# nintendops/DynamicFusion_Body

Measured on AMD Instinct MI355X. Metric: Mvoxels/s TSDF fusion + GN-iters/s warp solve, 256³ grid, 1/2/4/8 GPU, higher is better.
Workload: dtype f64 geometry / f32 volume

## Files before the change

### dynamicfusion_body_amd/csrc/dfh_integrate.hip

```cpp
#include "dfh_common.h"

#include <cstdlib>

namespace dfh {

template <typename T, int N>
struct alignas(sizeof(T) * N) Pack {
    T v[N];
};

struct IntegrateParams {
    Mat3 K, Kinv;
    Mat34 lw;
    double scale, cx, cy, cz, half, tdist, wmax;
    double Ax[4], Ay[4], Az[4], Ac[4];
    double inv_scale;
    float tdist_f, ts_f, wmax_f;
    int zp_shift;
    int planes_per_block;
    int X, Y, Z;
    int x0, nx;
    int H, W;
    int zpacks;
    const float *pyr;
    int pyr_off[6], pyr_w[6], pyr_h[6];
    int cull;
};

constexpr int kFixShift = 20;
constexpr int kFixOne = 1 << kFixShift;
constexpr int kFixHalf = 1 << (kFixShift - 1);
constexpr int kFixBand = 8;
constexpr int kFastMaxDim = 2048;
constexpr int kBrX = 4, kBrY = 2, kBrZ = 256 / (kBrX * kBrY);
constexpr int kMaxColumnBricks = 16;
constexpr int kPyrLevels = 5;
constexpr int kCullMargin = 1 << 10;
constexpr long kEarlyRowsMaxVoxels = 1L << 23;
constexpr long kTargetBlocks = 1L << 40;

template <typename DepthT, bool PINHOLE>
__device__ __forceinline__ bool exact_voxel(const IntegrateParams &p, const DepthT *__restrict__ depth,
                                            int x, int y, int z, double &sd_out) {
    const double *lw = p.lw.m;
    const double px = p.scale * ((double)x - p.half) + p.cx;
    const double py = p.scale * ((double)y - p.half) + p.cy;
    const double pz = p.scale * ((double)z - p.half) + p.cz;
    const double l0 = ((lw[0] * px + lw[1] * py) + lw[2] * pz) + lw[3];
    const double l1 = ((lw[4] * px + lw[5] * py) + lw[6] * pz) + lw[7];
    const double l2 = ((lw[8] * px + lw[9] * py) + lw[10] * pz) + lw[11];
    double p0, p1, p2;
    if (PINHOLE) {
        p0 = p.K.m[0] * l0 + p.K.m[2] * l2;
        p1 = p.K.m[4] * l1 + p.K.m[5] * l2;
        p2 = l2;
    } else {
        p0 = (p.K.m[0] * l0 + p.K.m[1] * l1) + p.K.m[2] * l2;
        p1 = (p.K.m[3] * l0 + p.K.m[4] * l1) + p.K.m[5] * l2;
        p2 = (p.K.m[6] * l0 + p.K.m[7] * l1) + p.K.m[8] * l2;
    }
    sd_out = 0.0;
    if (!(p2 != 0.0)) return false;
    const double u = p0 / p2;
    const double v = p1 / p2;
    if (!((u >= 0.0) && (u < (double)(p.W - 1)) && (v >= 0.0) && (v < (double)(p.H - 1)))) return false;
    const int ui = (int)rint(u);
    const int vi = (int)rint(v);
    const double zd = -1.0 * (double)depth[(size_t)vi * p.W + ui];
    if (!(zd > 0.0)) return false;
    double cz;
    if (PINHOLE) {
        cz = zd;
    } else {
        cz = (p.Kinv.m[6] * (zd * u) + p.Kinv.m[7] * (zd * v)) + p.Kinv.m[8] * (zd * 1.0);
    }
    const double sd = cz - l2;
    sd_out = sd;
    return sd > -1.0 * p.tdist;
}

template <typename DepthT, bool PINHOLE, bool LAZY>
__device__ __forceinline__ bool exact_voxel_rare(const IntegrateParams *pp, const DepthT *__restrict__ depth,
                                                 int x, int y, int z, double &sd_out) {
    asm volatile("" : "+v"(x), "+v"(y), "+v"(z));
    if (LAZY) asm volatile("" : "+s"(pp));
    return exact_voxel<DepthT, PINHOLE>(*pp, depth, x, y, z, sd_out);
}

__device__ __forceinline__ const IntegrateParams *kernarg_params(int byte_offset) {
    typedef const char __attribute__((address_space(4))) *KernArgBytes;
    KernArgBytes ka = (KernArgBytes)__builtin_amdgcn_kernarg_segment_ptr();
    return (const IntegrateParams *)(ka + byte_offset);
}
constexpr int kParamsAfterThreePointers = 24;

__device__ __forceinline__ double rcp_nr1(double d) {
    const double r = __builtin_amdgcn_rcp(d);
    return __builtin_fma(r, __builtin_fma(-d, r, 1.0), r);
}

__device__ __forceinline__ int cvt_i32_sat(double x) {
    int r;
    asm("v_cvt_i32_f64 %0, %1" : "=v"(r) : "v"(x));
    return r;
}

__device__ __forceinline__ void pack_coords(const IntegrateParams &p, int &y, int &zp) {
    const int lin = blockIdx.x * 256 + threadIdx.x;
    if (p.zp_shift >= 0) {
        y = lin >> p.zp_shift;
        zp = lin & ((1 << p.zp_shift) - 1);
    } else {
        y = lin / p.zpacks;
        zp = lin - y * p.zpacks;
    }
}

struct NoHook {
    __device__ __forceinline__ void operator()(bool) const {}
};

template <typename DepthT, int VEC, bool PINHOLE, bool STRIDED, bool LAZY = true, typename Hook = NoHook>
__device__ __forceinline__ bool view_pack(const IntegrateParams &p, const IntegrateParams *p_rare, const DepthT *__restrict__ depth, int x,
                                          int y, int z0, float (&ms)[VEC], bool (&upd)[VEC], Hook &&after_gathers = NoHook()) {
    constexpr int ZS = STRIDED ? 64 : 1;
    constexpr int NC = PINHOLE ? 3 : 4;
    const unsigned ulim = (unsigned)(p.W - 1) << kFixShift;
    const unsigned vlim = (unsigned)(p.H - 1) << kFixShift;
    double base[NC];
    {
        const double xf = (double)x, yf = (double)y, zf = (double)z0;
#pragma unroll
        for (int r = 0; r < NC; ++r)
            base[r] = __builtin_fma(p.Az[r], zf, __builtin_fma(p.Ax[r], xf, __builtin_fma(p.Ay[r], yf, p.Ac[r])));
    }
    const double p2_last = __builtin_fma(p.Az[2], (double)((VEC - 1) * ZS), base[2]);
    const bool pack_singular = !((fabs(base[2]) > 1e-6) & (fabs(p2_last) > 1e-6) & ((base[2] > 0.0) == (p2_last > 0.0)));

    double l2v[VEC];
    float l2f[VEC];
    unsigned pix[VEC];
    bool inside[VEC], amb[VEC];
    double rinv[VEC];
    if (VEC == 4) {
        double d[4];
#pragma unroll
        for (int j = 0; j < 4; ++j) d[j] = __builtin_fma(p.Az[2], (double)(j * ZS), base[2]);
        const double d01 = d[0] * d[1], d23 = d[2] * d[3];
        const double rall = rcp_nr1(d01 * d23);
        const double r01 = rall * d23, r23 = rall * d01;
        rinv[0] = r01 * d[1]; rinv[1] = r01 * d[0]; rinv[2 % VEC] = r23 * d[3 % VEC]; rinv[3 % VEC] = r23 * d[2 % VEC];
    } else {
#pragma unroll
        for (int j = 0; j < VEC; ++j) rinv[j] = rcp_nr1(__builtin_fma(p.Az[2], (double)(j * ZS), base[2]));
    }
#pragma unroll
    for (int j = 0; j < VEC; ++j) {
        const double jf = (double)(j * ZS);
        const double p0 = __builtin_fma(p.Az[0], jf, base[0]);
        const double p1 = __builtin_fma(p.Az[1], jf, base[1]);
        const double p2 = __builtin_fma(p.Az[2], jf, base[2]);
        l2v[j] = PINHOLE ? p2 : __builtin_fma(p.Az[NC - 1], jf, base[NC - 1]);
        l2f[j] = (float)l2v[j];
        const double r = rinv[j];
        const int qu = cvt_i32_sat(p0 * r);
        const int qv = cvt_i32_sat(p1 * r);
        const unsigned du = (unsigned)((qu + kFixBand) & (kFixHalf - 1));
        const unsigned dv = (unsigned)((qv + kFixBand) & (kFixHalf - 1));
        amb[j] = pack_singular | ((du < dv ? du : dv) <= 2u * kFixBand);
        inside[j] = ((unsigned)qu < ulim) & ((unsigned)qv < vlim);
        const int ui = (qu + kFixHalf) >> kFixShift;
        const int vi = (qv + kFixHalf) >> kFixShift;
        pix[j] = inside[j] ? (unsigned)(__mul24(vi, p.W) + ui) : 0u;
    }
    DepthT dval[VEC];
#pragma unroll
    for (int j = 0; j < VEC; ++j) dval[j] = depth[pix[j]];
    {
        bool any_inside = false;
#pragma unroll
        for (int j = 0; j < VEC; ++j) any_inside = any_inside | inside[j] | amb[j];
        after_gathers(any_inside);
    }
    bool any = false;
#pragma unroll
    for (int j = 0; j < VEC; ++j) {
        const float zdf = -(float)dval[j];
        const bool hit = inside[j] & (zdf > 0.0f);
        bool ok, redo, freespace;
        if (PINHOLE) {
            const float d32 = zdf - (l2f[j] - p.tdist_f);
            const float band = fmaf(fabsf(l2f[j]), 2e-6f, 1e-5f);
            ok = hit & (d32 > 0.0f);
            redo = amb[j] | (hit & (fabsf(d32) <= band));
            freespace = d32 > 2.0f * p.tdist_f + band;
        } else {
            ok = hit;
            redo = amb[j];
            freespace = false;
        }
        float m = p.ts_f;
        if (__builtin_expect(redo, 0)) {
            double sd;
            ok = exact_voxel_rare<DepthT, PINHOLE, LAZY>(p_rare, depth, x, y, z0 + j * ZS, sd);
            m = (float)((sd < p.tdist ? sd : p.tdist) * p.inv_scale);
        } else if (ok & !freespace) {
            double cz = -(double)dval[j];
            if (!PINHOLE) {
                const double jf = (double)(j * ZS);
                const double r = rcp_nr1(__builtin_fma(p.Az[2], jf, base[2])) * (1.0 / (double)kFixOne);
                const double u = __builtin_fma(p.Az[0], jf, base[0]) * r;
                const double v = __builtin_fma(p.Az[1], jf, base[1]) * r;
                cz = __builtin_fma(p.Kinv.m[6] * cz, u, __builtin_fma(p.Kinv.m[7] * cz, v, p.Kinv.m[8] * cz));
            }
            const double sd = cz - l2v[j];
            if (!PINHOLE) {
                const double margin = sd + p.tdist;
                ok = margin > 0.0;
                if (fabs(margin) < 1e-7) ok = exact_voxel_rare<DepthT, PINHOLE, LAZY>(p_rare, depth, x, y, z0 + j * ZS, cz);
            }
            m = (float)((sd < p.tdist ? sd : p.tdist) * p.inv_scale);
        }
        ok = ok & (z0 + j * ZS < p.Z);
        ms[j] = m;
        upd[j] = ok;
        any = any | ok;
    }
    return any;
}

template <int VEC>
__device__ __forceinline__ void apply_pack(Pack<float, VEC> &t, Pack<float, VEC> &w, const float (&ms)[VEC], const bool (&upd)[VEC],
                                           float wmax_f) {
#pragma unroll
    for (int j = 0; j < VEC; ++j) {
        const float wt = w.v[j];
        const float d = wt + 1.0f;
        const float n = fmaf(t.v[j], wt, ms[j]);
        const float r = __builtin_amdgcn_rcpf(d);
        float q = n * r;
        q = fmaf(fmaf(-d, q, n), r, q);
        t.v[j] = upd[j] ? q : t.v[j];
        w.v[j] = upd[j] ? fminf(d, wmax_f) : wt;
    }
}

template <typename DepthT, int VEC, bool PINHOLE, bool STRIDED>
__global__ __launch_bounds__(256) void integrate_depth_kernel(float *__restrict__ tsdf,
                                                               float *__restrict__ tsdf_w,
                                                               const DepthT *__restrict__ depth,
                                                               const IntegrateParams p) {
    int y, zp;
    pack_coords(p, y, zp);
    if (y >= p.Y) return;
    const int lane = threadIdx.x & 63;
    const int z0 = STRIDED ? (zp - lane) * VEC + lane : zp * VEC;
    constexpr int ZS = STRIDED ? 64 : 1;
    const int xl_end = min(p.nx, (int)(blockIdx.y + 1) * p.planes_per_block);
    for (int xl = blockIdx.y * p.planes_per_block; xl < xl_end; ++xl) {
        float ms[VEC];
        bool upd[VEC];
        if (!view_pack<DepthT, VEC, PINHOLE, STRIDED>(p, kernarg_params(kParamsAfterThreePointers), depth, p.x0 + xl, y, z0, ms, upd)) continue;
        const size_t off = ((size_t)xl * p.Y + y) * p.Z + z0;
        using P = Pack<float, VEC>;
        P t, w;
        if (STRIDED) {
#pragma unroll
            for (int j = 0; j < VEC; ++j) { t.v[j] = tsdf[off + j * ZS]; w.v[j] = tsdf_w[off + j * ZS]; }
        } else {
            t = *reinterpret_cast<const P *>(tsdf + off);
            w = *reinterpret_cast<const P *>(tsdf_w + off);
        }
        apply_pack<VEC>(t, w, ms, upd, p.wmax_f);
        if (STRIDED) {
#pragma unroll
            for (int j = 0; j < VEC; ++j) {
                if (upd[j]) { tsdf[off + j * ZS] = t.v[j]; tsdf_w[off + j * ZS] = w.v[j]; }
            }
        } else {
            *reinterpret_cast<P *>(tsdf + off) = t;
            *reinterpret_cast<P *>(tsdf_w + off) = w;
        }
    }
}

template <typename DepthT, bool PINHOLE>
__global__ __launch_bounds__(256) void integrate_depth_rows_early_kernel(float *__restrict__ tsdf, float *__restrict__ tsdf_w,
                                                                          const DepthT *__restrict__ depth, const IntegrateParams p) {
    int y, zp;
    pack_coords(p, y, zp);
    if (y >= p.Y) return;
    const int z0 = zp * 4;
    const int xl = blockIdx.y;
    float ms[4];
    bool upd[4];
    const size_t off = ((size_t)xl * p.Y + y) * p.Z + z0;
    using P = Pack<float, 4>;
    P t, w;
    bool loaded = false;
    const bool any = view_pack<DepthT, 4, PINHOLE, false>(p, kernarg_params(kParamsAfterThreePointers), depth, p.x0 + xl, y, z0, ms, upd, [&](bool any_inside) {
        if (any_inside) {
            t = *reinterpret_cast<const P *>(tsdf + off);
            w = *reinterpret_cast<const P *>(tsdf_w + off);
            loaded = true;
        }
    });
    if (!any) return;
    if (!loaded) {
        t = *reinterpret_cast<const P *>(tsdf + off);
        w = *reinterpret_cast<const P *>(tsdf_w + off);
    }
    apply_pack<4>(t, w, ms, upd, p.wmax_f);
    *reinterpret_cast<P *>(tsdf + off) = t;
    *reinterpret_cast<P *>(tsdf_w + off) = w;
}

constexpr int kMaxViews = 16;
struct ViewPtrs {
    const void *depth[kMaxViews];
    int n;
};

template <typename DepthT, int VEC, bool PINHOLE>
__global__ __launch_bounds__(256) void integrate_depth_multi_kernel(float *__restrict__ tsdf, float *__restrict__ tsdf_w,
                                                                     const IntegrateParams *__restrict__ views, const ViewPtrs vp) {
    int y, zp;
    pack_coords(views[0], y, zp);
    if (y >= views[0].Y) return;
    const int z0 = zp * VEC;
    const int nx = views[0].nx, ppb = views[0].planes_per_block;
    const int xl_end = min(nx, (int)(blockIdx.y + 1) * ppb);
    for (int xl = blockIdx.y * ppb; xl < xl_end; ++xl) {
        using P = Pack<float, VEC>;
        P t, w;
        bool loaded = false;
        const size_t off = ((size_t)xl * views[0].Y + y) * views[0].Z + z0;
        for (int v = 0; v < vp.n; ++v) {
            const IntegrateParams &p = views[v];
            float ms[VEC];
            bool upd[VEC];
            if (!view_pack<DepthT, VEC, PINHOLE, false, false>(p, &p, static_cast<const DepthT *>(vp.depth[v]), p.x0 + xl, y, z0, ms, upd)) continue;
            if (!loaded) {
                t = *reinterpret_cast<const P *>(tsdf + off);
                w = *reinterpret_cast<const P *>(tsdf_w + off);
                loaded = true;
            }
            apply_pack<VEC>(t, w, ms, upd, p.wmax_f);
        }
        if (loaded) {
            *reinterpret_cast<P *>(tsdf + off) = t;
            *reinterpret_cast<P *>(tsdf_w + off) = w;
        }
    }
}


struct BrickGeom {
    int nbz;
    int nyb;
    int nxb;
    int nzi;
    int nzc;
};

struct BrickBounds {
    int umin, umax, vmin, vmax;
    double l2min;
    bool front;
};

template <bool PINHOLE, int BY>
__device__ __forceinline__ void brick_corner(const IntegrateParams &p, int x0, int y0, int z0, int c, int &qu, int &qv, double &l2, bool &front) {
    constexpr int NC = PINHOLE ? 3 : 4;
    constexpr int BZ = 256 / (kBrX * BY);
    const double xf = (double)(x0 + ((c & 1) ? kBrX - 1 : 0)), yf = (double)(y0 + ((c & 2) ? BY - 1 : 0)), zf = (double)(z0 + ((c & 4) ? BZ - 1 : 0));
    double q[NC];
#pragma unroll
    for (int r = 0; r < NC; ++r) q[r] = __builtin_fma(p.Az[r], zf, __builtin_fma(p.Ax[r], xf, __builtin_fma(p.Ay[r], yf, p.Ac[r])));
    front = q[2] > 1e-6;
    const double rr = rcp_nr1(q[2]);
    qu = cvt_i32_sat(q[0] * rr);
    qv = cvt_i32_sat(q[1] * rr);
    l2 = q[NC - 1];
}

template <bool PINHOLE>
__device__ __forceinline__ bool bounds_culled(const IntegrateParams &p, BrickBounds b) {
    if (!b.front) return false;
    int umin = b.umin, umax = b.umax, vmin = b.vmin, vmax = b.vmax;
    const int ulim = (p.W - 1) << kFixShift, vlim = (p.H - 1) << kFixShift;
    if (umax < -kCullMargin || umin > ulim + kCullMargin || vmax < -kCullMargin || vmin > vlim + kCullMargin) return true;
    if (!PINHOLE || p.pyr == nullptr) return false;
    umin = max(umin, -2 * kFixOne); vmin = max(vmin, -2 * kFixOne);
    umax = min(umax, ulim + 2 * kFixOne); vmax = min(vmax, vlim + 2 * kFixOne);
    int px0 = (umin - kCullMargin) >> kFixShift, px1 = (umax + kCullMargin + kFixOne - 1) >> kFixShift;
    int py0 = (vmin - kCullMargin) >> kFixShift, py1 = (vmax + kCullMargin + kFixOne - 1) >> kFixShift;
    px0 = max(px0, 0); py0 = max(py0, 0); px1 = min(px1, p.W - 1); py1 = min(py1, p.H - 1);
    if (px1 < px0 || py1 < py0) return false;
    int L = 1;
    while (L <= kPyrLevels && (((px1 >> L) - (px0 >> L)) > 1 || ((py1 >> L) - (py0 >> L)) > 1)) ++L;
    if (L > kPyrLevels) {
        L = kPyrLevels;
        if (((px1 >> L) - (px0 >> L)) > 3 || ((py1 >> L) - (py0 >> L)) > 3) return false;
    }
    const float *lv = p.pyr + p.pyr_off[L];
    const int wl = p.pyr_w[L];
    const int cx0 = px0 >> L, cx1 = px1 >> L, cy0 = py0 >> L, cy1 = py1 >> L;
    float zmax = 0.0f;
    for (int cy = cy0; cy <= cy1; ++cy)
        for (int cx = cx0; cx <= cx1; ++cx) zmax = fmaxf(zmax, lv[cy * wl + cx]);
    const float l2f = (float)b.l2min;
    return zmax + p.tdist_f + fmaf(fabsf(l2f), 4e-7f, 1e-5f) <= l2f;
}

template <bool PINHOLE, int BY>
__device__ __forceinline__ bool brick_culled(const IntegrateParams &p, int x0, int y0, int z0) {
    BrickBounds b{0x7fffffff, (int)0x80000000, 0x7fffffff, (int)0x80000000, __builtin_huge_val(), true};
#pragma unroll
    for (int c = 0; c < 8; ++c) {
        int qu, qv;
        double l2;
        bool fr;
        brick_corner<PINHOLE, BY>(p, x0, y0, z0, c, qu, qv, l2, fr);
        b.front = b.front && fr;
        b.umin = min(b.umin, qu); b.umax = max(b.umax, qu); b.vmin = min(b.vmin, qv); b.vmax = max(b.vmax, qv);
        b.l2min = fmin(b.l2min, l2);
    }
    return bounds_culled<PINHOLE>(p, b);
}

template <bool PINHOLE, bool BYVAL, int BY>
__global__ __launch_bounds__(256) void brick_classify_kernel(const IntegrateParams *__restrict__ views, const IntegrateParams p1,
                                                              int n_views, const BrickGeom g, int n_bricks,
                                                              unsigned short *__restrict__ mask) {
    constexpr int BZ = 256 / (kBrX * BY);
    const int b = blockIdx.x * 256 + threadIdx.x;
    if (b >= n_bricks) return;
    const int bz = b % g.nbz;
    const int t = b / g.nbz;
    const int by = t % g.nyb;
    const int bx = t / g.nyb;
    unsigned m = 0;
    for (int v = 0; v < n_views; ++v) {
        const IntegrateParams &p = BYVAL ? p1 : views[v];
        if (!(p.cull && brick_culled<PINHOLE, BY>(p, p.x0 + kBrX * bx, BY * by, BZ * bz))) m |= 1u << v;
    }
    mask[b] = (unsigned short)m;
}

typedef float f32x4 __attribute__((ext_vector_type(4)));
static_assert(sizeof(f32x4) == sizeof(Pack<float, 4>), "a pack is one 16-byte access");

template <bool NT>
__device__ __forceinline__ Pack<float, 4> ld_pack(const float *a) {
    const f32x4 v = NT ? __builtin_nontemporal_load(reinterpret_cast<const f32x4 *>(a)) : *reinterpret_cast<const f32x4 *>(a);
    Pack<float, 4> r;
    r.v[0] = v.x; r.v[1] = v.y; r.v[2] = v.z; r.v[3] = v.w;
    return r;
}
template <bool NT>
__device__ __forceinline__ void st_pack(float *a, const Pack<float, 4> &r) {
    f32x4 v;
    v.x = r.v[0]; v.y = r.v[1]; v.z = r.v[2]; v.w = r.v[3];
    if (NT) __builtin_nontemporal_store(v, reinterpret_cast<f32x4 *>(a));
    else *reinterpret_cast<f32x4 *>(a) = v;
}

template <int BY>
struct ColumnLane {
    static constexpr int BZ = 256 / (kBrX * BY), BZP = BZ / 4;
    int xl, y, zl, bz0;
    bool in_xy;
    size_t row;
    unsigned mv;

    __device__ __forceinline__ unsigned long long init(const BrickGeom &g, int nx, int Y, int Z, const unsigned short *__restrict__ mask,
                                                       unsigned full_mask, bool all) {
        const int lane = threadIdx.x & 63;
        const int wv = __builtin_amdgcn_readfirstlane((int)(threadIdx.x >> 6));
        const int by = blockIdx.x, c = blockIdx.y, bx = blockIdx.z;
        xl = kBrX * bx + lane / (BY * BZP);
        y = BY * by + (lane / BZP) % BY;
        zl = 4 * (lane % BZP);
        bz0 = 4 * c * g.nzi + wv;
        in_xy = xl < nx && y < Y;
        row = ((size_t)xl * Y + y) * Z;
        const int bz = bz0 + 4 * lane;
        const bool mine = lane < g.nzi && bz < g.nbz;
        mv = 0;
        if (mine) mv = mask ? (unsigned)mask[(size_t)(bx * g.nyb + by) * g.nbz + bz] : full_mask;
        return __ballot(all ? mine : mv != 0);
    }

    __device__ __forceinline__ int z_of(int i) const { return BZ * (bz0 + 4 * i) + zl; }
};

#ifndef DFH_K1_GF_WAVES
#define DFH_K1_GF_WAVES 7
#endif
#ifdef DFH_K1_WAVES
#define DFH_K1_OCC __attribute__((amdgpu_waves_per_eu(DFH_K1_WAVES, DFH_K1_WAVES)))
#else
#define DFH_K1_OCC __attribute__((amdgpu_waves_per_eu(GATHER_FIRST && PINHOLE ? DFH_K1_GF_WAVES : 1)))
#endif
template <typename DepthT, bool PINHOLE, int BY, bool PREFETCH, bool NT, bool GATHER_FIRST>
__global__ __launch_bounds__(256) DFH_K1_OCC void integrate_depth_column_kernel(float *__restrict__ tsdf, float *__restrict__ tsdf_w,
                                                                      const DepthT *__restrict__ depth, const IntegrateParams p,
                                                                      const BrickGeom g, const unsigned short *__restrict__ mask) {
    ColumnLane<BY> c;
    unsigned long long alive = c.init(g, p.nx, p.Y, p.Z, mask, 1u, false);
    if (alive == 0) return;
    using P = Pack<float, 4>;
    const IntegrateParams *p_rare = kernarg_params(kParamsAfterThreePointers);
    int i = __builtin_ctzll(alive);
    alive &= alive - 1;
    int z0 = c.z_of(i);
    bool in_grid = c.in_xy && z0 < p.Z;
    P t, w;
    if (GATHER_FIRST) {
        float ms[4];
        bool upd[4];
        bool any = view_pack<DepthT, 4, PINHOLE, false>(p, p_rare, depth, p.x0 + c.xl, c.y, z0, ms, upd) && in_grid;
        while (alive) {
            P tb, wb;
            if (any) { tb = ld_pack<NT>(tsdf + c.row + z0); wb = ld_pack<NT>(tsdf_w + c.row + z0); }
            const int zn = c.z_of(__builtin_ctzll(alive));
            alive &= alive - 1;
            float msn[4];
            bool updn[4];
            const bool anyn = view_pack<DepthT, 4, PINHOLE, false>(p, p_rare, depth, p.x0 + c.xl, c.y, zn, msn, updn, [&](bool) {
                if (any) {
                    apply_pack<4>(tb, wb, ms, upd, p.wmax_f);
                    st_pack<NT>(tsdf + c.row + z0, tb);
                    st_pack<NT>(tsdf_w + c.row + z0, wb);
                }
            }) && c.in_xy && zn < p.Z;
#pragma unroll
            for (int j = 0; j < 4; ++j) { ms[j] = msn[j]; upd[j] = updn[j]; }
            any = anyn;
            z0 = zn;
        }
        if (any) {
            t = ld_pack<NT>(tsdf + c.row + z0);
            w = ld_pack<NT>(tsdf_w + c.row + z0);
            apply_pack<4>(t, w, ms, upd, p.wmax_f);
            st_pack<NT>(tsdf + c.row + z0, t);
            st_pack<NT>(tsdf_w + c.row + z0, w);
        }
        return;
    }
    if (PREFETCH && in_grid) { t = ld_pack<NT>(tsdf + c.row + z0); w = ld_pack<NT>(tsdf_w + c.row + z0); }
    for (;;) {
        if (!PREFETCH && in_grid) { t = ld_pack<NT>(tsdf + c.row + z0); w = ld_pack<NT>(tsdf_w + c.row + z0); }
        const bool more = alive != 0;
        int zn = 0;
        bool in_grid_n = false;
        P tn, wn;
        if (more) {
            zn = c.z_of(__builtin_ctzll(alive));
            in_grid_n = c.in_xy && zn < p.Z;
        }
        float ms[4];
        bool upd[4];
        const bool any = view_pack<DepthT, 4, PINHOLE, false>(p, p_rare, depth, p.x0 + c.xl, c.y, z0, ms, upd, [&](bool) {
            if (PREFETCH && in_grid_n) { tn = ld_pack<NT>(tsdf + c.row + zn); wn = ld_pack<NT>(tsdf_w + c.row + zn); }
        });
        if (any && in_grid) {
            apply_pack<4>(t, w, ms, upd, p.wmax_f);
            st_pack<NT>(tsdf + c.row + z0, t);
            st_pack<NT>(tsdf_w + c.row + z0, w);
        }
        if (!more) break;
        alive &= alive - 1;
        z0 = zn;
        in_grid = in_grid_n;
        if (PREFETCH) { t = tn; w = wn; }
    }
}

template <typename DepthT, bool PINHOLE, int BY, bool FRESH, bool NT>
__global__ __launch_bounds__(256) void integrate_depth_multi_column_kernel(float *__restrict__ tsdf, float *__restrict__ tsdf_w,
                                                                            const IntegrateParams *__restrict__ views, const ViewPtrs vp,
                                                                            const BrickGeom g, const unsigned short *__restrict__ mask,
                                                                            const float fresh_t) {
    ColumnLane<BY> c;
    const int nx = views[0].nx, Y = views[0].Y, Z = views[0].Z;
    unsigned long long alive = c.init(g, nx, Y, Z, mask, (1u << vp.n) - 1u, FRESH);
    using P = Pack<float, 4>;
    while (alive) {
        const int i = __builtin_ctzll(alive);
        alive &= alive - 1;
        unsigned m = (unsigned)__builtin_amdgcn_readlane((int)c.mv, i);
        const int z0 = c.z_of(i);
        const bool in_grid = c.in_xy && z0 < Z;
        P t, w;
        if (FRESH) {
#pragma unroll
            for (int j = 0; j < 4; ++j) { t.v[j] = fresh_t; w.v[j] = 0.0f; }
        } else if (in_grid) {
            t = ld_pack<NT>(tsdf + c.row + z0);
            w = ld_pack<NT>(tsdf_w + c.row + z0);
        }
        bool touched = FRESH;
        while (m) {
            const int v = __builtin_ctz(m);
            m &= m - 1;
            const IntegrateParams &p = views[v];
            float ms[4];
            bool upd[4];
            const bool any = view_pack<DepthT, 4, PINHOLE, false, false>(p, &p, static_cast<const DepthT *>(vp.depth[v]), p.x0 + c.xl, c.y, z0, ms, upd);
            if (!(any && in_grid)) continue;
            apply_pack<4>(t, w, ms, upd, p.wmax_f);
            touched = true;
        }
        if (touched && in_grid) {
            st_pack<NT>(tsdf + c.row + z0, t);
            st_pack<NT>(tsdf_w + c.row + z0, w);
        }
    }
}

template <typename T>
__global__ __launch_bounds__(256) void fill_pair_kernel(T *__restrict__ a, T va, T *__restrict__ b, T vb, size_t n) {
    for (size_t i = (size_t)blockIdx.x * 256 + threadIdx.x; i < n; i += (size_t)gridDim.x * 256) { a[i] = va; b[i] = vb; }
}

constexpr int kParamChunk = 6;
struct ParamChunk {
    IntegrateParams v[kParamChunk];
};
static_assert(sizeof(IntegrateParams) % 8 == 0 && sizeof(ParamChunk) + 24 <= 4096, "the chunk must fit the kernel-argument segment");
__global__ __launch_bounds__(256) void upload_params_kernel(IntegrateParams *dst, const ParamChunk c, int n) {
    typedef const unsigned long long __attribute__((address_space(4))) *KernArgWords;
    KernArgWords ka = (KernArgWords)__builtin_amdgcn_kernarg_segment_ptr() + 1;
    unsigned long long *out = reinterpret_cast<unsigned long long *>(dst);
    const int words = n * (int)(sizeof(IntegrateParams) / 8);
    for (int i = threadIdx.x; i < words; i += 256) out[i] = ka[i];
    (void)c;
}

struct PyrViews {
    const void *depth[kMaxViews];
    float *pyr[kMaxViews];
};

template <typename DepthT>
__global__ __launch_bounds__(256) void depth_pyramid_kernel(const PyrViews pv, int H, int W, const IntegrateParams p1) {
    const DepthT *__restrict__ depth = static_cast<const DepthT *>(pv.depth[blockIdx.z]);
    float *__restrict__ pyr = pv.pyr[blockIdx.z];
    __shared__ float s[256];
    const int t = threadIdx.x;
    const int qx = t & 15, qy = t >> 4;
    const int px = 32 * (int)blockIdx.x + 2 * qx, py = 32 * (int)blockIdx.y + 2 * qy;
    auto zval = [&](int x, int y) {
        if (x >= W || y >= H) return 0.0f;
        const float z = -(float)depth[(size_t)y * W + x];
        return z > 0.0f ? z : 0.0f;
    };
    float m = fmaxf(fmaxf(zval(px, py), zval(px + 1, py)), fmaxf(zval(px, py + 1), zval(px + 1, py + 1)));
    {
        const int cx = 16 * (int)blockIdx.x + qx, cy = 16 * (int)blockIdx.y + qy;
        if (cx < p1.pyr_w[1] && cy < p1.pyr_h[1]) pyr[p1.pyr_off[1] + cy * p1.pyr_w[1] + cx] = m;
    }
    s[t] = m;
    __syncthreads();
    int n = 16;
#pragma unroll
    for (int L = 2; L <= kPyrLevels; ++L) {
        const int h = n >> 1;
        float v = 0.0f;
        const int x = t % h, y = t / h;
        if (t < h * h) v = fmaxf(fmaxf(s[(2 * y) * n + 2 * x], s[(2 * y) * n + 2 * x + 1]), fmaxf(s[(2 * y + 1) * n + 2 * x], s[(2 * y + 1) * n + 2 * x + 1]));
        __syncthreads();
        if (t < h * h) {
            s[y * h + x] = v;
            const int cx = h * (int)blockIdx.x + x, cy = h * (int)blockIdx.y + y;
            if (cx < p1.pyr_w[L] && cy < p1.pyr_h[L]) pyr[p1.pyr_off[L] + cy * p1.pyr_w[L] + cx] = v;
        }
        __syncthreads();
        n = h;
    }
}

static size_t pyramid_floats(int H, int W, int *off, int *pw, int *ph) {
    size_t tot = 0;
    for (int L = 1; L <= kPyrLevels; ++L) {
        const int wl = (W + (1 << L) - 1) >> L, hl = (H + (1 << L) - 1) >> L;
        if (off) { off[L] = (int)tot; pw[L] = wl; ph[L] = hl; }
        tot += (size_t)wl * hl;
    }
    return (tot + 3) / 4 * 4;
}

struct OclParams {
    float proj[12], kinv2[3], tdist, wmax;
    int X, Y, Z, x0, nx, H, W;
};

__global__ __launch_bounds__(256) void integrate_depth_ocl_kernel(float *__restrict__ tsdf, float *__restrict__ tsdf_w,
                                                                   const float *__restrict__ depth, const OclParams p) {
// ... 87 lines not shown
        if (strided) {
            if constexpr (VEC == 4) {
                if (pinhole) {
                    hipLaunchKernelGGL((integrate_depth_kernel<DepthT, 4, true, true>), grid, block, 0, stream,
                                       (float *)tsdf, (float *)tsdf_w, (const DepthT *)depth, p);
                } else {
                    hipLaunchKernelGGL((integrate_depth_kernel<DepthT, 4, false, true>), grid, block, 0, stream,
                                       (float *)tsdf, (float *)tsdf_w, (const DepthT *)depth, p);
                }
            }
        } else if (VEC == 4 && p.planes_per_block == 1 && (long)p.nx * p.Y * p.Z <= kEarlyRowsMaxVoxels && !on(opt().k1_late_loads)) {
            if (pinhole)
                hipLaunchKernelGGL((integrate_depth_rows_early_kernel<DepthT, true>), grid, block, 0, stream, (float *)tsdf, (float *)tsdf_w,
                                   (const DepthT *)depth, p);
            else
                hipLaunchKernelGGL((integrate_depth_rows_early_kernel<DepthT, false>), grid, block, 0, stream, (float *)tsdf, (float *)tsdf_w,
                                   (const DepthT *)depth, p);
        } else if (pinhole) {
            hipLaunchKernelGGL((integrate_depth_kernel<DepthT, VEC, true, false>), grid, block, 0, stream,
                               (float *)tsdf, (float *)tsdf_w, (const DepthT *)depth, p);
        } else {
            hipLaunchKernelGGL((integrate_depth_kernel<DepthT, VEC, false, false>), grid, block, 0, stream,
                               (float *)tsdf, (float *)tsdf_w, (const DepthT *)depth, p);
        }
    } else {
        if (pinhole) {
            hipLaunchKernelGGL((integrate_depth_exact_kernel<VolT, DepthT, VEC, true>), grid, block, 0, stream,
                               (VolT *)tsdf, (VolT *)tsdf_w, (const DepthT *)depth, p);
        } else {
            hipLaunchKernelGGL((integrate_depth_exact_kernel<VolT, DepthT, VEC, false>), grid, block, 0, stream,
                               (VolT *)tsdf, (VolT *)tsdf_w, (const DepthT *)depth, p);
        }
    }
    DFH_HIP_CHECK(hipGetLastError());
    return DFH_OK;
}

static void fold_affine(IntegrateParams &p) {
    const double *lw = p.lw.m;
    const double *K = p.K.m;
    const double off[3] = {p.cx - p.scale * p.half, p.cy - p.scale * p.half, p.cz - p.scale * p.half};
    double L[3][4];
    for (int r = 0; r < 3; ++r) {
        for (int c = 0; c < 3; ++c) L[r][c] = lw[4 * r + c] * p.scale;
        L[r][3] = lw[4 * r + 0] * off[0] + lw[4 * r + 1] * off[1] + lw[4 * r + 2] * off[2] + lw[4 * r + 3];
    }
    for (int r = 0; r < 3; ++r) {
        double row[4];
        for (int c = 0; c < 4; ++c) row[c] = K[3 * r + 0] * L[0][c] + K[3 * r + 1] * L[1][c] + K[3 * r + 2] * L[2][c];
        p.Ax[r] = row[0]; p.Ay[r] = row[1]; p.Az[r] = row[2]; p.Ac[r] = row[3];
    }
    p.Ax[3] = L[2][0]; p.Ay[3] = L[2][1]; p.Az[3] = L[2][2]; p.Ac[3] = L[2][3];
    for (int r = 0; r < 2; ++r) {
        p.Ax[r] *= (double)kFixOne; p.Ay[r] *= (double)kFixOne; p.Az[r] *= (double)kFixOne; p.Ac[r] *= (double)kFixOne;
    }
    p.inv_scale = 1.0 / p.scale;
    p.tdist_f = (float)p.tdist;
    p.ts_f = (float)(p.tdist * p.inv_scale);
    p.wmax_f = (float)p.wmax;
}

static bool fill_params(IntegrateParams &p, const int res[3], int tsdf_res, int x0, int x1, int H, int W, const double K[9],
                        const double Kinv[9], const double lw[12], double scale, const double center[3], double tdist,
                        double wmax, bool vec4) {
    for (int i = 0; i < 9; ++i) { p.K.m[i] = K[i]; p.Kinv.m[i] = Kinv[i]; }
    for (int i = 0; i < 12; ++i) p.lw.m[i] = lw[i];
    p.scale = scale; p.cx = center[0]; p.cy = center[1]; p.cz = center[2];
    p.half = (double)tsdf_res / 2.0;
    p.tdist = tdist; p.wmax = wmax;
    p.X = res[0]; p.Y = res[1]; p.Z = res[2];
    p.x0 = x0; p.nx = x1 - x0; p.H = H; p.W = W;
    p.zpacks = vec4 ? res[2] / 4 : res[2];
    p.zp_shift = -1;
    for (int b = 0; b < 31; ++b) if (p.zpacks == (1 << b)) p.zp_shift = b;
    p.pyr = nullptr; p.cull = 0;
    for (int l = 0; l < 6; ++l) { p.pyr_off[l] = 0; p.pyr_w[l] = 0; p.pyr_h[l] = 0; }
    fold_affine(p);
    {
        const long per_plane_blocks = ((long)p.Y * p.zpacks + 255) / 256;
        long chunks = (kTargetBlocks + per_plane_blocks - 1) / per_plane_blocks;
        if (chunks < 1) chunks = 1;
        if (chunks > p.nx) chunks = p.nx;
        p.planes_per_block = (int)((p.nx + chunks - 1) / chunks);
        if (opt().k1_planes_per_block > 0) p.planes_per_block = (int)opt().k1_planes_per_block;
    }
    return K[1] == 0.0 && K[3] == 0.0 && K[6] == 0.0 && K[7] == 0.0 && K[8] == 1.0 && Kinv[6] == 0.0 && Kinv[7] == 0.0 &&
           Kinv[8] == 1.0;
}

}

namespace dfh {

static size_t params_bytes(int n_views) { return ((size_t)n_views * sizeof(IntegrateParams) + 15) / 16 * 16; }

static void attach_pyramid(IntegrateParams &p, void *workspace, int n_views, int view, int H, int W) {
    const size_t pf = pyramid_floats(H, W, p.pyr_off, p.pyr_w, p.pyr_h);
    p.pyr = reinterpret_cast<const float *>(static_cast<char *>(workspace) + params_bytes(n_views)) + (size_t)view * pf;
}

template <typename DepthT>
static int launch_pyramids(const void *const *depth, int n_views, int H, int W, const IntegrateParams *hp, hipStream_t s) {
    PyrViews pv;
    for (int v = 0; v < n_views; ++v) { pv.depth[v] = depth[v]; pv.pyr[v] = const_cast<float *>(hp[v].pyr); }
    dim3 grid((unsigned)((W + 31) / 32), (unsigned)((H + 31) / 32), (unsigned)n_views);
    hipLaunchKernelGGL(depth_pyramid_kernel<DepthT>, grid, dim3(256), 0, s, pv, H, W, hp[0]);
    DFH_HIP_CHECK(hipGetLastError());
    return DFH_OK;
}

static BrickGeom brick_geom(int by_shape, int Y, int Z, int nx, dim3 &grid, int &n_bricks) {
    BrickGeom g;
    const int bz_len = 256 / (kBrX * by_shape);
    g.nbz = (Z + bz_len - 1) / bz_len;
    g.nyb = (Y + by_shape - 1) / by_shape;
    g.nxb = (nx + kBrX - 1) / kBrX;
    const int per_col = (g.nbz + 3) / 4;
    int nzi = per_col < kMaxColumnBricks ? per_col : kMaxColumnBricks;
    while (nzi > 1 && (long)g.nyb * g.nxb * ((per_col + nzi - 1) / nzi) < 8192) nzi = (nzi + 1) / 2;
    if (opt().k1_nzi > 0) nzi = (int)(opt().k1_nzi < kMaxColumnBricks ? opt().k1_nzi : kMaxColumnBricks);
    g.nzi = nzi;
    g.nzc = (per_col + nzi - 1) / nzi;
    grid = dim3((unsigned)g.nyb, (unsigned)g.nzc, (unsigned)g.nxb);
    n_bricks = g.nbz * g.nyb * g.nxb;
    return g;
}

static bool use_nt(size_t slab_voxels) {
    if (opt().k1_nt >= 0) return opt().k1_nt != 0;
    return slab_voxels * 8 > ((size_t)256 << 20);
}

static size_t pyr_bytes(int n_views, int H, int W) { return (size_t)n_views * pyramid_floats(H, W, nullptr, nullptr, nullptr) * sizeof(float); }

}

namespace dfh {

struct K1Plan {
    int path;
    bool bricks;
    bool cull;
    bool gather_first;
};

static K1Plan single_view_plan(int vol_dtype, const int res[3], int x0, int x1, bool fast_ok, bool vec4, bool have_ws) {
    if (vol_dtype != DFH_F32 || !fast_ok) return {DFH_K1_PATH_EXACT, false, false, false};
    const long slab_voxels = (long)(x1 - x0) * res[1] * res[2];
    const long bricks_min = opt().k1_bricks_min >= 0 ? opt().k1_bricks_min : kEarlyRowsMaxVoxels / 256 + 1;
    const long slab_bricks = (long)((res[1] + 3) / 4) * ((res[2] + 15) / 16) * ((x1 - x0 + kBrX - 1) / kBrX);
    if (vec4 && !on(opt().k1_no_bricks) && slab_bricks >= bricks_min) {
        const bool want_cull = !on(opt().k1_bricks_nocull) && (opt().k1_cull >= 0 ? opt().k1_cull != 0 : (size_t)slab_voxels * 8 > ((size_t)256 << 20));
        if (!want_cull || have_ws) {
            const bool gf = opt().k1_gather_first >= 0 ? opt().k1_gather_first != 0 : !want_cull;
            return {gf ? DFH_K1_PATH_ROWS : want_cull ? DFH_K1_PATH_COLUMNS_CULLED : DFH_K1_PATH_COLUMNS, true, want_cull, gf};
        }
    }
    return {DFH_K1_PATH_ROWS, false, false, false};
}

}

extern "C" size_t dfh_integrate_workspace_bytes(int n_views, int H, int W, const int res[3], int x0, int x1) {
    if (n_views <= 0 || H < 2 || W < 2 || !res || res[1] <= 0 || res[2] <= 0 || x1 < x0) return 0;
    dim3 grid;
    int n_bricks = 0;
    dfh::brick_geom(dfh::kBrY, res[1], res[2], x1 - x0, grid, n_bricks);
    return dfh::params_bytes(n_views) + dfh::pyr_bytes(n_views, H, W) + ((size_t)n_bricks * sizeof(unsigned short) + 15) / 16 * 16;
}

extern "C" int dfh_integrate_depth_path(int vol_dtype, const int res[3], int x0, int x1, int H, int W, int have_workspace) {
    using namespace dfh;
    DFH_REQUIRE(res && res[0] > 0 && res[1] > 0 && res[2] > 0 && 0 <= x0 && x0 <= x1 && x1 <= res[0], "dfh_integrate_depth_path: bad grid or slab");
    const bool fast_ok = H <= kFastMaxDim && W <= kFastMaxDim;
    const bool vec4 = res[2] % 4 == 0 && !on(opt().k1_force_scalar);
    return single_view_plan(vol_dtype, res, x0, x1, fast_ok, vec4, have_workspace != 0).path;
}

extern "C" int dfh_integrate_depth(void *tsdf, void *tsdf_w, int vol_dtype, const int res[3],
                                   int tsdf_res, int x0, int x1, const void *depth, int depth_dtype,
                                   int H, int W, const double K[9], const double Kinv[9],
                                   const double lw[12], double scale, const double center[3],
                                   double tdist, double wmax, void *workspace, size_t workspace_bytes, void *stream) {
    using namespace dfh;
    DFH_REQUIRE(tsdf && tsdf_w && depth && res && K && Kinv && lw && center, "dfh_integrate_depth: null pointer");
    DFH_REQUIRE(vol_dtype == DFH_F32 || vol_dtype == DFH_F64, "dfh_integrate_depth: bad vol_dtype %d", vol_dtype);
    DFH_REQUIRE(depth_dtype == DFH_F32 || depth_dtype == DFH_F64, "dfh_integrate_depth: bad depth_dtype %d", depth_dtype);
    DFH_REQUIRE(res[0] > 0 && res[1] > 0 && res[2] > 0, "dfh_integrate_depth: bad grid %dx%dx%d", res[0], res[1], res[2]);
    DFH_REQUIRE(0 <= x0 && x0 <= x1 && x1 <= res[0], "dfh_integrate_depth: slab [%d,%d) outside [0,%d)", x0, x1, res[0]);
    DFH_REQUIRE(H >= 2 && W >= 2, "dfh_integrate_depth: depth map %dx%d too small", H, W);
    DFH_REQUIRE((long)H * W < (1L << 31), "dfh_integrate_depth: depth map too large");
    DFH_REQUIRE(x1 - x0 <= 65535, "dfh_integrate_depth: slab has more than 65535 planes");
    if (x1 == x0) return DFH_OK;

    IntegrateParams p;
    const size_t esz = vol_dtype == DFH_F32 ? 4 : 8;
    const bool vec4 = (res[2] % 4 == 0) && ((uintptr_t)tsdf % (4 * esz) == 0) && ((uintptr_t)tsdf_w % (4 * esz) == 0) &&
                      !on(opt().k1_force_scalar);
    const bool pinhole = fill_params(p, res, tsdf_res, x0, x1, H, W, K, Kinv, lw, scale, center, tdist, wmax, vec4);
    hipStream_t s = static_cast<hipStream_t>(stream);
    const bool fast_ok = H <= kFastMaxDim && W <= kFastMaxDim && scale > 0.0 && tdist > 0.0;

    const bool have_ws = workspace && workspace_bytes >= dfh_integrate_workspace_bytes(1, H, W, res, x0, x1);
    const K1Plan plan = single_view_plan(vol_dtype, res, x0, x1, fast_ok, vec4, have_ws);
    if (plan.bricks) {
        const bool cull = plan.cull, gf = plan.gather_first;
        dim3 grid;
        int n_bricks = 0;
        const BrickGeom g = brick_geom(kBrY, p.Y, p.Z, p.nx, grid, n_bricks);
        unsigned short *mask = nullptr;
        if (cull) {
            p.cull = 1;
            attach_pyramid(p, workspace, 1, 0, H, W);
            const void *dptr[1] = {depth};
            const int rc = depth_dtype == DFH_F32 ? launch_pyramids<float>(dptr, 1, H, W, &p, s) : launch_pyramids<double>(dptr, 1, H, W, &p, s);
            if (rc != DFH_OK) return rc;
            mask = reinterpret_cast<unsigned short *>(static_cast<char *>(workspace) + params_bytes(1) + pyr_bytes(1, H, W));
            const dim3 cgrid((unsigned)((n_bricks + 255) / 256));
#define DFH_CLASSIFY(PH, BY) hipLaunchKernelGGL((brick_classify_kernel<PH, true, BY>), cgrid, dim3(256), 0, s, nullptr, p, 1, g, n_bricks, mask)
            if (pinhole) DFH_CLASSIFY(true, kBrY); else DFH_CLASSIFY(false, kBrY);
#undef DFH_CLASSIFY
        }
        const bool prefetch = opt().k1_prefetch >= 0 ? opt().k1_prefetch != 0 : cull;
        const bool nt = use_nt((size_t)p.nx * p.Y * p.Z);
#define DFH_COL(DT, PH, BY, PF, NT, GF) hipLaunchKernelGGL((integrate_depth_column_kernel<DT, PH, BY, PF, NT, GF>), grid, dim3(256), 0, s, (float *)tsdf, (float *)tsdf_w, (const DT *)depth, p, g, mask)
#define DFH_COL_PF(DT, PH, BY, NT) do { if (gf) DFH_COL(DT, PH, BY, false, NT, true); else if (prefetch) DFH_COL(DT, PH, BY, true, NT, false); else DFH_COL(DT, PH, BY, false, NT, false); } while (0)
#define DFH_COL_SHAPE(DT, PH) do { if (nt) DFH_COL_PF(DT, PH, kBrY, true); else DFH_COL_PF(DT, PH, kBrY, false); } while (0)
        if (depth_dtype == DFH_F32) { if (pinhole) DFH_COL_SHAPE(float, true); else DFH_COL_SHAPE(float, false); }
        else { if (pinhole) DFH_COL_SHAPE(double, true); else DFH_COL_SHAPE(double, false); }
#undef DFH_COL_SHAPE
#undef DFH_COL_PF
#undef DFH_COL
        DFH_HIP_CHECK(hipGetLastError());
        return DFH_OK;
    }

#define DFH_DISPATCH(VT, DT, FAST)                                                            \
    return vec4 ? launch_integrate<VT, DT, 4, FAST>(tsdf, tsdf_w, depth, p, pinhole, s)       \
                : launch_integrate<VT, DT, 1, FAST>(tsdf, tsdf_w, depth, p, pinhole, s)
    if (vol_dtype == DFH_F32) {
        if (fast_ok) {
            if (depth_dtype == DFH_F32) { DFH_DISPATCH(float, float, true); }
            DFH_DISPATCH(float, double, true);
        }
        if (depth_dtype == DFH_F32) { DFH_DISPATCH(float, float, false); }
        DFH_DISPATCH(float, double, false);
    }
    if (depth_dtype == DFH_F32) { DFH_DISPATCH(double, float, false); }
    DFH_DISPATCH(double, double, false);
#undef DFH_DISPATCH
}

extern "C" size_t dfh_integrate_multi_workspace_bytes(int n_views) {
    return n_views > 0 ? dfh::params_bytes(n_views) : 0;
}

static int integrate_multi_fill(void *tsdf, void *tsdf_w, int vol_dtype, const int res[3], int x0, int x1, double fresh_value, void *stream) {
    using namespace dfh;
    DFH_REQUIRE(tsdf && tsdf_w && res, "dfh_integrate_depth_multi_fresh: null pointer");
    DFH_REQUIRE(vol_dtype == DFH_F32 || vol_dtype == DFH_F64, "dfh_integrate_depth_multi_fresh: bad vol_dtype %d", vol_dtype);
    DFH_REQUIRE(res[0] > 0 && res[1] > 0 && res[2] > 0 && 0 <= x0 && x0 <= x1 && x1 <= res[0], "dfh_integrate_depth_multi_fresh: bad grid or slab");
    const size_t n = (size_t)(x1 - x0) * res[1] * res[2];
    if (n == 0) return DFH_OK;
    const unsigned nb = (unsigned)((n + 255) / 256 < 65536 * 16 ? (n + 255) / 256 : 65536 * 16);
    if (vol_dtype == DFH_F32)
        hipLaunchKernelGGL(fill_pair_kernel<float>, dim3(nb), dim3(256), 0, (hipStream_t)stream, (float *)tsdf, (float)fresh_value, (float *)tsdf_w, 0.0f, n);
    else
        hipLaunchKernelGGL(fill_pair_kernel<double>, dim3(nb), dim3(256), 0, (hipStream_t)stream, (double *)tsdf, fresh_value, (double *)tsdf_w, 0.0, n);
    DFH_HIP_CHECK(hipGetLastError());
    return DFH_OK;
}

static int integrate_multi_impl(void *tsdf, void *tsdf_w, int vol_dtype, const int res[3], int tsdf_res, int x0, int x1,
                                int n_views, const void *const *depth, int depth_dtype, int H, int W,
                                const double K[9], const double Kinv[9], const double *lw, double scale,
                                const double center[3], double tdist, double wmax, void *workspace,
                                size_t workspace_bytes, void *stream, bool fresh, double fresh_value) {
    using namespace dfh;
    DFH_REQUIRE(n_views >= 0 && n_views <= kMaxViews, "dfh_integrate_depth_multi: %d views (at most %d per call)", n_views, kMaxViews);
    if (n_views == 0) return fresh ? integrate_multi_fill(tsdf, tsdf_w, vol_dtype, res, x0, x1, fresh_value, stream) : DFH_OK;
    DFH_REQUIRE(tsdf && tsdf_w && depth && res && K && Kinv && lw && center, "dfh_integrate_depth_multi: null pointer");
    for (int v = 0; v < n_views; ++v) DFH_REQUIRE(depth[v], "dfh_integrate_depth_multi: depth map %d is null", v);
    DFH_REQUIRE(vol_dtype == DFH_F32 || vol_dtype == DFH_F64, "dfh_integrate_depth_multi: bad vol_dtype %d", vol_dtype);
    DFH_REQUIRE(depth_dtype == DFH_F32 || depth_dtype == DFH_F64, "dfh_integrate_depth_multi: bad depth_dtype %d", depth_dtype);
    const size_t esz = vol_dtype == DFH_F32 ? 4 : 8;
    const bool vec4 = res[0] > 0 && res[1] > 0 && res[2] > 0 && (res[2] % 4 == 0) && ((uintptr_t)tsdf % (4 * esz) == 0) &&
                      ((uintptr_t)tsdf_w % (4 * esz) == 0) && !on(opt().k1_force_scalar);
    const bool fast_ok = vol_dtype == DFH_F32 && H <= kFastMaxDim && W <= kFastMaxDim && scale > 0.0 && tdist > 0.0 &&
                         workspace && workspace_bytes >= dfh_integrate_multi_workspace_bytes(n_views) && !on(opt().k1_no_multi);
    if (!fast_ok || n_views == 1 || x1 <= x0) {
        if (fresh) {
            const int rc = integrate_multi_fill(tsdf, tsdf_w, vol_dtype, res, x0, x1, fresh_value, stream);
            if (rc != DFH_OK) return rc;
        }
        for (int v = 0; v < n_views; ++v) {
            const int rc = dfh_integrate_depth(tsdf, tsdf_w, vol_dtype, res, tsdf_res, x0, x1, depth[v], depth_dtype, H, W, K, Kinv,
                                               lw + 12 * v, scale, center, tdist, wmax, workspace, workspace_bytes, stream);
            if (rc != DFH_OK) return rc;
        }
        return DFH_OK;
    }
    DFH_REQUIRE(res[0] > 0 && res[1] > 0 && res[2] > 0, "dfh_integrate_depth_multi: bad grid %dx%dx%d", res[0], res[1], res[2]);
    DFH_REQUIRE(0 <= x0 && x0 <= x1 && x1 <= res[0], "dfh_integrate_depth_multi: slab [%d,%d) outside [0,%d)", x0, x1, res[0]);
    DFH_REQUIRE(H >= 2 && W >= 2 && (long)H * W < (1L << 31), "dfh_integrate_depth_multi: bad depth map size %dx%d", H, W);
    DFH_REQUIRE(x1 - x0 <= 65535, "dfh_integrate_depth_multi: slab has more than 65535 planes");
    IntegrateParams hp[kMaxViews];
    ViewPtrs vp;
// ... 103 lines not shown
```

Measured before the change: 507,200.

## Skip depth gathers for out-of-view waves and split view_pack into uniform passes

Restructures view_pack so each wave ballots whether any lane projects inside the image or is ambiguous, and skips the depth gathers and SDF evaluation entirely when none does. Per-voxel work is split into separate valid and rare-redo passes, the ambiguity test is rewritten with shifted unsigned compares, and pixel offsets are computed as 32-bit byte offsets. The weight update uses paired float vectors, and the gather-first path addresses the TSDF through 32-bit byte offsets, guarded in the planner by a slab-size limit. The changes aim to cut divergent per-lane branching, address arithmetic, and wasted memory traffic for voxels outside the view, at the cost of an extra ballot and more complex control flow.

```diff
diff --git a/dynamicfusion_body_amd/csrc/dfh_integrate.hip b/dynamicfusion_body_amd/csrc/dfh_integrate.hip
--- a/dynamicfusion_body_amd/csrc/dfh_integrate.hip
+++ b/dynamicfusion_body_amd/csrc/dfh_integrate.hip
@@ -137,111 +137,153 @@
     const double p2_last = __builtin_fma(p.Az[2], (double)((VEC - 1) * ZS), base[2]);
     const bool pack_singular = !((fabs(base[2]) > 1e-6) & (fabs(p2_last) > 1e-6) & ((base[2] > 0.0) == (p2_last > 0.0)));
 
+    const auto at = [&](int r, int j) -> double { return j == 0 ? base[r] : __builtin_fma(p.Az[r], (double)(j * ZS), base[r]); };
     double l2v[VEC];
     float l2f[VEC];
-    unsigned pix[VEC];
+    unsigned pixb[VEC];
     bool inside[VEC], amb[VEC];
     double rinv[VEC];
     if (VEC == 4) {
         double d[4];
 #pragma unroll
-        for (int j = 0; j < 4; ++j) d[j] = __builtin_fma(p.Az[2], (double)(j * ZS), base[2]);
+        for (int j = 0; j < 4; ++j) d[j] = at(2, j);
         const double d01 = d[0] * d[1], d23 = d[2] * d[3];
         const double rall = rcp_nr1(d01 * d23);
         const double r01 = rall * d23, r23 = rall * d01;
         rinv[0] = r01 * d[1]; rinv[1] = r01 * d[0]; rinv[2 % VEC] = r23 * d[3 % VEC]; rinv[3 % VEC] = r23 * d[2 % VEC];
     } else {
 #pragma unroll
-        for (int j = 0; j < VEC; ++j) rinv[j] = rcp_nr1(__builtin_fma(p.Az[2], (double)(j * ZS), base[2]));
+        for (int j = 0; j < VEC; ++j) rinv[j] = rcp_nr1(at(2, j));
     }
 #pragma unroll
     for (int j = 0; j < VEC; ++j) {
-        const double jf = (double)(j * ZS);
-        const double p0 = __builtin_fma(p.Az[0], jf, base[0]);
-        const double p1 = __builtin_fma(p.Az[1], jf, base[1]);
-        const double p2 = __builtin_fma(p.Az[2], jf, base[2]);
-        l2v[j] = PINHOLE ? p2 : __builtin_fma(p.Az[NC - 1], jf, base[NC - 1]);
+        const double p0 = at(0, j);
+        const double p1 = at(1, j);
+        const double p2 = at(2, j);
+        l2v[j] = PINHOLE ? p2 : __builtin_fma(p.Az[NC - 1], (double)(j * ZS), base[NC - 1]);
         l2f[j] = (float)l2v[j];
         const double r = rinv[j];
         const int qu = cvt_i32_sat(p0 * r);
         const int qv = cvt_i32_sat(p1 * r);
-        const unsigned du = (unsigned)((qu + kFixBand) & (kFixHalf - 1));
-        const unsigned dv = (unsigned)((qv + kFixBand) & (kFixHalf - 1));
-        amb[j] = pack_singular | ((du < dv ? du : dv) <= 2u * kFixBand);
+        const unsigned au = (unsigned)qu + kFixHalf, av = (unsigned)qv + kFixHalf;
+        constexpr int kBandShift = 32 - (kFixShift - 1);
+        const unsigned du = (au << kBandShift) + ((unsigned)kFixBand << kBandShift);
+        const unsigned dv = (av << kBandShift) + ((unsigned)kFixBand << kBandShift);
+        amb[j] = pack_singular | ((du < dv ? du : dv) < ((2u * kFixBand + 1u) << kBandShift));
         inside[j] = ((unsigned)qu < ulim) & ((unsigned)qv < vlim);
-        const int ui = (qu + kFixHalf) >> kFixShift;
-        const int vi = (qv + kFixHalf) >> kFixShift;
-        pix[j] = inside[j] ? (unsigned)(__mul24(vi, p.W) + ui) : 0u;
-    }
+        const unsigned pb = (__umul24(av >> kFixShift, (unsigned)p.W) + (au >> kFixShift)) * (unsigned)sizeof(DepthT);
+        pixb[j] = inside[j] ? pb : 0u;
+        asm("" : "+v"(pixb[j]));
+    }
+    bool any_inside = false;
+#pragma unroll
+    for (int j = 0; j < VEC; ++j) any_inside = any_inside | inside[j] | amb[j];
+    const bool wave_in = __builtin_amdgcn_ballot_w64(any_inside) != 0;
     DepthT dval[VEC];
-#pragma unroll
-    for (int j = 0; j < VEC; ++j) dval[j] = depth[pix[j]];
-    {
-        bool any_inside = false;
-#pragma unroll
-        for (int j = 0; j < VEC; ++j) any_inside = any_inside | inside[j] | amb[j];
-        after_gathers(any_inside);
-    }
-    bool any = false;
+    if (wave_in) {
+#pragma unroll
+        for (int j = 0; j < VEC; ++j) dval[j] = *reinterpret_cast<const DepthT *>(reinterpret_cast<const char *>(depth) + pixb[j]);
+    }
+    after_gathers(any_inside);
+    if (!wave_in) {
+#pragma unroll
+        for (int j = 0; j < VEC; ++j) { ms[j] = p.ts_f; upd[j] = false; }
+        return false;
+    }
+    bool ok[VEC], redo[VEC], val[VEC];
+    bool any_val = false, any_redo = false;
 #pragma unroll
     for (int j = 0; j < VEC; ++j) {
         const float zdf = -(float)dval[j];
         const bool hit = inside[j] & (zdf > 0.0f);
-        bool ok, redo, freespace;
         if (PINHOLE) {
             const float d32 = zdf - (l2f[j] - p.tdist_f);
             const float band = fmaf(fabsf(l2f[j]), 2e-6f, 1e-5f);
-            ok = hit & (d32 > 0.0f);
-            redo = amb[j] | (hit & (fabsf(d32) <= band));
-            freespace = d32 > 2.0f * p.tdist_f + band;
+            const bool freespace = d32 > 2.0f * p.tdist_f + band;
+            ok[j] = hit & (d32 > 0.0f);
+            redo[j] = amb[j] | (hit & (fabsf(d32) <= band));
+            val[j] = ok[j] & !redo[j] & !freespace;
         } else {
-            ok = hit;
-            redo = amb[j];
-            freespace = false;
-        }
-        float m = p.ts_f;
-        if (__builtin_expect(redo, 0)) {
-            double sd;
-            ok = exact_voxel_rare<DepthT, PINHOLE, LAZY>(p_rare, depth, x, y, z0 + j * ZS, sd);
-            m = (float)((sd < p.tdist ? sd : p.tdist) * p.inv_scale);
-        } else if (ok & !freespace) {
-            double cz = -(double)dval[j];
-            if (!PINHOLE) {
+            ok[j] = hit;
+            redo[j] = amb[j];
+            val[j] = ok[j] & !redo[j];
+        }
+        ms[j] = p.ts_f;
+        any_val = any_val | val[j];
+        any_redo = any_redo | redo[j];
+    }
+    if (any_val) {
+#pragma unroll
+        for (int j = 0; j < VEC; ++j) {
+            if (PINHOLE) {
+                const double sd = -(double)dval[j] - l2v[j];
+                const float m = (float)(__builtin_fmin(sd, p.tdist) * p.inv_scale);
+                ms[j] = val[j] ? m : ms[j];
+            } else if (val[j]) {
+                double cz = -(double)dval[j];
                 const double jf = (double)(j * ZS);
                 const double r = rcp_nr1(__builtin_fma(p.Az[2], jf, base[2])) * (1.0 / (double)kFixOne);
                 const double u = __builtin_fma(p.Az[0], jf, base[0]) * r;
                 const double v = __builtin_fma(p.Az[1], jf, base[1]) * r;
                 cz = __builtin_fma(p.Kinv.m[6] * cz, u, __builtin_fma(p.Kinv.m[7] * cz, v, p.Kinv.m[8] * cz));
+                const double sd = cz - l2v[j];
+                const double margin = sd + p.tdist;
+                ok[j] = margin > 0.0;
+                if (fabs(margin) < 1e-7) ok[j] = exact_voxel_rare<DepthT, PINHOLE, LAZY>(p_rare, depth, x, y, z0 + j * ZS, cz);
+                ms[j] = (float)((sd < p.tdist ? sd : p.tdist) * p.inv_scale);
             }
-            const double sd = cz - l2v[j];
-            if (!PINHOLE) {
-                const double margin = sd + p.tdist;
-                ok = margin > 0.0;
-                if (fabs(margin) < 1e-7) ok = exact_voxel_rare<DepthT, PINHOLE, LAZY>(p_rare, depth, x, y, z0 + j * ZS, cz);
+        }
+    }
+    if (__builtin_expect(any_redo, 0)) {
+#pragma unroll
+        for (int j = 0; j < VEC; ++j) {
+            if (redo[j]) {
+                double sd;
+                ok[j] = exact_voxel_rare<DepthT, PINHOLE, LAZY>(p_rare, depth, x, y, z0 + j * ZS, sd);
+                ms[j] = (float)((sd < p.tdist ? sd : p.tdist) * p.inv_scale);
             }
-            m = (float)((sd < p.tdist ? sd : p.tdist) * p.inv_scale);
-        }
-        ok = ok & (z0 + j * ZS < p.Z);
-        ms[j] = m;
-        upd[j] = ok;
-        any = any | ok;
+        }
+    }
+    bool any = false;
+    const int zleft = p.Z - z0;
+#pragma unroll
+    for (int j = 0; j < VEC; ++j) {
+        upd[j] = ok[j] & (j * ZS < zleft);
+        any = any | upd[j];
     }
     return any;
 }
 
+typedef float f32x2 __attribute__((ext_vector_type(2)));
 template <int VEC>
 __device__ __forceinline__ void apply_pack(Pack<float, VEC> &t, Pack<float, VEC> &w, const float (&ms)[VEC], const bool (&upd)[VEC],
                                            float wmax_f) {
-#pragma unroll
-    for (int j = 0; j < VEC; ++j) {
-        const float wt = w.v[j];
+    static_assert(VEC % 2 == 0 || VEC == 1, "pairs of voxels");
+    if constexpr (VEC == 1) {
+        const float wt = w.v[0];
         const float d = wt + 1.0f;
-        const float n = fmaf(t.v[j], wt, ms[j]);
+        const float n = fmaf(t.v[0], wt, ms[0]);
         const float r = __builtin_amdgcn_rcpf(d);
         float q = n * r;
         q = fmaf(fmaf(-d, q, n), r, q);
-        t.v[j] = upd[j] ? q : t.v[j];
-        w.v[j] = upd[j] ? fminf(d, wmax_f) : wt;
+        t.v[0] = upd[0] ? q : t.v[0];
+        w.v[0] = upd[0] ? fminf(d, wmax_f) : wt;
+    } else {
+#pragma unroll
+    for (int j = 0; j < VEC; j += 2) {
+        const f32x2 wt = {w.v[j], w.v[j + 1]};
+        const f32x2 tt = {t.v[j], t.v[j + 1]};
+        const f32x2 m = {ms[j], ms[j + 1]};
+        const f32x2 d = wt + 1.0f;
+        const f32x2 n = __builtin_elementwise_fma(tt, wt, m);
+        const f32x2 r = {__builtin_amdgcn_rcpf(d.x), __builtin_amdgcn_rcpf(d.y)};
+        f32x2 q = n * r;
+        q = __builtin_elementwise_fma(__builtin_elementwise_fma(-d, q, n), r, q);
+        t.v[j] = upd[j] ? q.x : t.v[j];
+        t.v[j + 1] = upd[j + 1] ? q.y : t.v[j + 1];
+        w.v[j] = upd[j] ? fminf(d.x, wmax_f) : wt.x;
+        w.v[j + 1] = upd[j + 1] ? fminf(d.y, wmax_f) : wt.y;
+    }
     }
 }
 
@@ -518,12 +560,15 @@
     bool in_grid = c.in_xy && z0 < p.Z;
     P t, w;
     if (GATHER_FIRST) {
+        const unsigned rowb = (unsigned)c.row * 4u;
+        const auto tp = [&](int z) { return reinterpret_cast<float *>(reinterpret_cast<char *>(tsdf) + (rowb + 4u * (unsigned)z)); };
+        const auto wp = [&](int z) { return reinterpret_cast<float *>(reinterpret_cast<char *>(tsdf_w) + (rowb + 4u * (unsigned)z)); };
         float ms[4];
         bool upd[4];
         bool any = view_pack<DepthT, 4, PINHOLE, false>(p, p_rare, depth, p.x0 + c.xl, c.y, z0, ms, upd) && in_grid;
         while (alive) {
             P tb, wb;
-            if (any) { tb = ld_pack<NT>(tsdf + c.row + z0); wb = ld_pack<NT>(tsdf_w + c.row + z0); }
+            if (any) { tb = ld_pack<NT>(tp(z0)); wb = ld_pack<NT>(wp(z0)); }
             const int zn = c.z_of(__builtin_ctzll(alive));
             alive &= alive - 1;
             float msn[4];
@@ -531,8 +576,8 @@
             const bool anyn = view_pack<DepthT, 4, PINHOLE, false>(p, p_rare, depth, p.x0 + c.xl, c.y, zn, msn, updn, [&](bool) {
                 if (any) {
                     apply_pack<4>(tb, wb, ms, upd, p.wmax_f);
-                    st_pack<NT>(tsdf + c.row + z0, tb);
-                    st_pack<NT>(tsdf_w + c.row + z0, wb);
+                    st_pack<NT>(tp(z0), tb);
+                    st_pack<NT>(wp(z0), wb);
                 }
             }) && c.in_xy && zn < p.Z;
 #pragma unroll
@@ -541,11 +586,11 @@
             z0 = zn;
         }
         if (any) {
-            t = ld_pack<NT>(tsdf + c.row + z0);
-            w = ld_pack<NT>(tsdf_w + c.row + z0);
+            t = ld_pack<NT>(tp(z0));
+            w = ld_pack<NT>(wp(z0));
             apply_pack<4>(t, w, ms, upd, p.wmax_f);
-            st_pack<NT>(tsdf + c.row + z0, t);
-            st_pack<NT>(tsdf_w + c.row + z0, w);
+            st_pack<NT>(tp(z0), t);
+            st_pack<NT>(wp(z0), w);
         }
         return;
     }
@@ -939,7 +984,7 @@
     if (vec4 && !on(opt().k1_no_bricks) && slab_bricks >= bricks_min) {
         const bool want_cull = !on(opt().k1_bricks_nocull) && (opt().k1_cull >= 0 ? opt().k1_cull != 0 : (size_t)slab_voxels * 8 > ((size_t)256 << 20));
         if (!want_cull || have_ws) {
-            const bool gf = opt().k1_gather_first >= 0 ? opt().k1_gather_first != 0 : !want_cull;
+            const bool gf = (opt().k1_gather_first >= 0 ? opt().k1_gather_first != 0 : !want_cull) && (size_t)slab_voxels * 4 <= 0xFFFFFFFFu;
             return {gf ? DFH_K1_PATH_ROWS : want_cull ? DFH_K1_PATH_COLUMNS_CULLED : DFH_K1_PATH_COLUMNS, true, want_cull, gf};
         }
     }
```

After: 508,100 (median of 6 runs). About the same (+0.2%).
